# tomasjakab/imm

Hardware: AMD Instinct MI355X
Metric: training images/sec at 128x128 K=10 (higher is better)
Workload: dtype bf16; 1 GPU; BASELINE configs[1] (N>1: configs[2]): CelebA-shape 128x128 K=10 IMM training step (fwd + VGG16 perceptual loss + bwd + clip + Adam), batch 32 per GPU; global_batch=32, image_size=128, n_maps=10, parallelism=dp1, hip_graph=True, weights=seeded random init; synthetic VGG16 (vgg16.caffemodel.h5 unavailable offline)

## Files before the change

imm_amd/_lib.py:

```python
import ctypes as C
import os

import torch

_HERE = os.path.dirname(os.path.abspath(__file__))
LIB_PATH = os.environ.get('IMM_HIP_LIB') or os.path.join(_HERE, 'libimm_hip.so')

IMM_BF16, IMM_F16, IMM_F32 = 0, 1, 2
CONV_BIAS, CONV_RELU, CONV_STATS, CONV_MASK, CONV_OUT_F32 = 1, 2, 4, 8, 16
SSE_BLOCKS = 512
OPTIMIZERS = {'adam': 0, 'adadelta': 1, 'adagrad': 2}
GAUSS_MODES = {'rot': 0, 'flat': 1, 'ankush': 2}
ABI_VERSION = 25


class ImmHipError(RuntimeError):
    pass


class ConvDesc(C.Structure):
    _fields_ = [(n, C.c_int32) for n in (
        'batch', 'hi', 'wi', 'ci', 'ldx', 'ho', 'wo', 'co', 'ldy', 'kh', 'kw', 'stride', 'pad_t', 'pad_l',
        'updiv', 'kpad', 'flags', 'ldmask', 'out_scale', 'out_off_y', 'out_off_x')]


class WgradJob(C.Structure):
    _fields_ = [('desc', ConvDesc), ('x', C.c_void_p), ('dy', C.c_void_p), ('slab', C.c_void_p), ('lddy', C.c_int32),
                ('nsplit', C.c_int32), ('x_scale', C.c_void_p), ('x_shift', C.c_void_p), ('x_relu', C.c_int32),
# ... 97 lines not shown
    'imm_masked_sse': [_P, _P, _I, _I, _I, _I, _P, _I, _I, _P, _P],
    'imm_masked_sse_f32': [_P, _I, _P, _I, _I, _I, _I, _P, _I, _P, _P],
    'imm_perceptual_finalize': [_P, _I, _P, _P, _I, _P, _I, _I, _P, _P, _P],
    'imm_cost_ema': [_P, _P, _F, _P],
    'imm_rms16': [_P, _L, _I, _P, _I, _P, _P],
    'imm_tap_grad': [_P, _I, _P, _P, _I, _I, _I, _I, _P, _I, _P, _I, _I, _I, _P],
    'imm_weight_decay_loss': [_P, _P, _P, _P, _I, _P, _P, _P, _P],
    'imm_clip_adam_step': [_P, _P, _P, _P, _P, _P, _P, _I, _I, _P, _P, _P, _P, _P, _P, _P, C.POINTER(OptHParams), _P, _P],
}

_SIGS_ALIGN = {
    'imm_align_coeffs': [_P, _P, _I, _I, _I, _P, _P],
    'imm_align_warp_u8': [_P, _I, _P, _P, _I, _P, _P, _P, _P, _I, _I, _I, _I, _P, _I, _P],
}

_SIGS64 = {
    'imm_conv2d_workspace_bytes': [C.POINTER(ConvDesc)],
    'imm_conv2d_group_workspace_bytes': [_P, _I],
    'imm_conv2d_wgrad_workspace_bytes': [C.POINTER(ConvDesc), _I, _I],
    'imm_conv2d_wgrad_multi_table_bytes': [_I],
    'imm_colsum_workspace_bytes': [_L, _I],
    'imm_bn_bwd_workspace_bytes': [_L, _I],
    'imm_upsample2x_bwd_bn_workspace_bytes': [_I, _I, _I, _I],
    'imm_masked_sse_workspace_bytes': [_I],
    'imm_vgg_head_scratch_bytes': [_I, _I],
}

_lib = None


def declared_symbols():
    return sorted(list(_SIGS) + list(_SIGS64) + ['imm_last_error', 'imm_source_digest'])


def alignment_symbols():
    return sorted(_SIGS_ALIGN)


def load():
    global _lib
    if _lib is not None:
        return _lib
    if not os.path.exists(LIB_PATH):
        raise ImmHipError('libimm_hip.so not found at %s: build it with `python imm_amd/build.py` '
                          '(there is no CPU fallback for the product path)' % LIB_PATH)
    if 'IMM_HIP_LIB' not in os.environ and os.path.isdir(os.path.join(_HERE, 'csrc')):
        from . import build as _b
        want, have = _b.source_digest(), _b.library_digest(LIB_PATH)
        if want != have:
            if not _b.have_compiler():
                raise ImmHipError('libimm_hip.so is stale (built from sources %s.., checkout is %s..) and hipcc is not '
                                  'available to rebuild it' % (have[:12] or '?', want[:12]))
            _b.build(verbose=False)
    lib = C.CDLL(LIB_PATH)
    for name in ('imm_last_error', 'imm_source_digest'):
        getattr(lib, name).restype = C.c_char_p
        getattr(lib, name).argtypes = []
    for name, args in list(_SIGS.items()) + list(_SIGS_ALIGN.items()):
        fn = getattr(lib, name)
        fn.argtypes = args
        fn.restype = C.c_int
    for name, args in _SIGS64.items():
        fn = getattr(lib, name)
        fn.argtypes = args
        fn.restype = C.c_int64
    v = lib.imm_abi_version()
    if v != ABI_VERSION:
        raise ImmHipError('libimm_hip.so ABI %d != expected %d' % (v, ABI_VERSION))
    _lib = lib
    return lib


def check(rc, what):
# ... 9 lines not shown
```

imm_amd/csrc/conv_common.h:

```cpp
#pragma once
#include "common.h"

struct ConvArgs {
  const uint16_t* x;
  const uint16_t* wt;
  const float* bias;
  void* y;
  float* stats;
  const uint16_t* mask;
  int M, hi, wi, ci8, ldx;
  int ho, wo, co, ldy;
  int kh, kw, stride, pad_t, pad_l, updiv;
  int kpad, KT, ntaps;
  int flags, ldmask;
  int n_nblk, n_blocks;
  int oscale, ooff_y, ooff_x;
  uint32_t x_bytes, wt_bytes;
  const uint16_t* tap_gt;
  const float* tap_lmask;
  const float* tap_coef;
  int tap_idx, tap_S, tap_l1;
};
#define IMM_CONV_TAP_ 0x20


#define IMM_CONV_GROUP_MAX 4
struct ConvArgsGroup {
  ConvArgs a[IMM_CONV_GROUP_MAX];
  int first[IMM_CONV_GROUP_MAX + 1];
  int n;
};

template <typename ET, int BM, int BN, int WGM, int WGN, int MT, int NT>
__device__ __forceinline__ void conv_epilogue(const ConvArgs& a, f32x4_t (&acc)[MT][NT], int tid, int wm, int wn, int m0,
                                              int n0, int mblk, float* red) {
  constexpr int TM = BM / WGM, TN = BN / WGN;
  const int lane = tid & 63;
  if (a.flags & IMM_DBG_NO_EPILOGUE) {
// ... 119 lines not shown
```

imm_amd/csrc/conv_hdeep.hip:

```cpp
#include "conv_common.h"
#include <stdlib.h>
#include <stdio.h>

typedef __attribute__((address_space(3))) void lds_void_t;
typedef __attribute__((ext_vector_type(4))) unsigned int u32x4_t;

#define HD_PW 16
#define HD_HW (HD_PW + 2)
#define HD_SLOTS(PH) (((PH) + 2) * HD_HW)
#define HD_HINSTR(PH) ((HD_SLOTS(PH) + 7) / 8)
#define HD_HSTAGE(PH) (HD_HINSTR(PH) * 64)
#define HD_OOB 0x80000000u

struct HdArgs {
  ConvArgs c;
  int n_patches, patches_x, patches_y;
  int n_wg;
  int n_img;
  unsigned long long* prof;
};

__device__ __forceinline__ void hd_dma16(u32x4_t rsrc, uint32_t lds_addr, uint32_t voff, uint32_t soff) {
  asm volatile("s_mov_b32 m0, %0\n\ts_nop 0\n\tbuffer_load_dwordx4 %1, %2, %3 offen lds"
               :: "s"(lds_addr), "v"(voff), "s"(rsrc), "s"(soff) : "memory");
// ... 7 lines not shown
template <int V> struct HdInt { static constexpr int value = V; };

__device__ __forceinline__ float hd_row_sum16(float x) {
  float y;
  asm volatile("s_nop 1\n\tv_add_f32_dpp %0, %1, %1 row_ror:8 row_mask:0xf bank_mask:0xf\n\t"
               "s_nop 1\n\tv_add_f32_dpp %0, %0, %0 row_ror:4 row_mask:0xf bank_mask:0xf\n\t"
               "s_nop 1\n\tv_add_f32_dpp %0, %0, %0 row_ror:2 row_mask:0xf bank_mask:0xf\n\t"
               "s_nop 1\n\tv_add_f32_dpp %0, %0, %0 row_ror:1 row_mask:0xf bank_mask:0xf\n\ts_nop 1"
               : "=&v"(y) : "v"(x));
  return y;
}

#ifndef IMM_HD_ROLL
#define IMM_HD_ROLL 1
#endif
template <typename ET, int BN, int NW, int PH, bool MAP8 = false, int NSB_ = 0, bool PERSIST = false, bool ROW3 = false, bool S2D = false>
__global__ __launch_bounds__(NW * 64) void conv_hdeep_kernel(const HdArgs ha) {
  const ConvArgs& a = ha.c;
  constexpr bool COL = IMM_HD_ROLL && ROW3 && !S2D && !MAP8;
  static_assert(!S2D || (!MAP8 && !PERSIST && NW == 4 && BN == 64), "stride-2 data gradient: 8x16 class patches x 64 channels, one tile per workgroup");
  constexpr int NCLS = S2D ? 4 : 1;
  static_assert((NW == 8 && PH == 16) || (NW == 4 && PH == 8), "wave (wm, wn) owns patch rows 4wm..4wm+3 x BN/2 channels");
  static_assert(!MAP8 || NW == 4, "two 8x8 images per 4-wave workgroup");
  static_assert(!(PERSIST && MAP8), "persistent tiles: 16x16 / 8x16 patches only");
  static_assert(!ROW3 || (NSB_ == 9 && !PERSIST), "row-at-a-time schedule: nine tap stages, one tile per workgroup");
  constexpr int HD_NSB = NSB_ ? NSB_ : MAP8 ? 3 : 4;
  constexpr int NPIECE = MAP8 ? 7 : 6;
  constexpr int TN = BN / 2, MT = 4, NT = TN / 16;
  constexpr int B_I = BN / (8 * NW);
  constexpr int SLOTS = MAP8 ? 200 : HD_SLOTS(PH);
  constexpr int HINSTR = (SLOTS + 7) / 8, HSTAGE = HINSTR * 64;
  static_assert(B_I >= 1 && NPIECE * NW >= HINSTR && (ROW3 || NPIECE <= 11 - HD_NSB), "halo pieces per wave cover the halo and land in time");
  constexpr int STEP_I = MAP8 ? 160 : (HD_HW * 128) / 16, STEP_KY = MAP8 ? 80 : (HD_HW * 128) / 16;
// ... 261 lines not shown
      ++t;
    }
  }
  HD_STAMP(4);
  if (!have_next) {
    asm volatile("s_waitcnt lgkmcnt(0)" ::: "memory");
    asm volatile("s_waitcnt vmcnt(0)" ::: "memory");
    __syncthreads();
  } else {
    asm volatile("s_waitcnt vmcnt(0)" ::: "memory");
  }
  HD_STAMP(5);
  const int img = e_img, y0 = e_y0, x0 = e_x0, n0 = e_n0, patch = e_patch;

  const bool f_relu = a.flags & IMM_CONV_RELU;
  const bool f_stats = !PERSIST && (a.flags & IMM_CONV_STATS), f_mask = a.flags & IMM_CONV_MASK;
  const int nb = n0 + wn * TN + q * (4 * NT);
  float s1[NT][4], s2[NT][4];
#pragma unroll
  for (int j = 0; j < NT; ++j)
#pragma unroll
    for (int r = 0; r < 4; ++r) { s1[j][r] = 0.f; s2[j][r] = 0.f; }
  if (have_next) load_bias(n_n0);
  const int64_t m_first = MAP8 ? ((int64_t)(img + wm) * 8 + (frow >> 3)) * 8 + (frow & 7)
                               : ((int64_t)img * a.ho + y0 + wm * 4) * a.wo + x0 + frow;
  const int64_t m_step = MAP8 ? 16 : a.wo;
  const bool rows_exist = !MAP8 || img + wm < ha.n_img;
  typedef short s16x2_t __attribute__((ext_vector_type(2)));
  typedef unsigned short u16x2_t __attribute__((ext_vector_type(2)));
  const s16x2_t zero2 = {0, 0}, one2 = {1, 1};
  if constexpr (S2D) {
// ... 36 lines not shown
          const int j = 2 * h + (e >> 1), r = (e & 1) * 2;
          v[2 * e] = acc[0][i][j][r]; v[2 * e + 1] = acc[0][i][j][r + 1];
        }
        unpack8<ET>(*(const uint4*)(a.mask + m * a.ldmask + nb + 8 * h), fp);
        unpack8<ET>(*(const uint4*)(a.tap_gt + m * a.ldmask + nb + 8 * h), fg);
#pragma unroll
        for (int e = 0; e < 8; ++e) {
          float d = fp[e] - fg[e];
          if (a.tap_l1) d = d > 0.f ? 1.f : (d < 0.f ? -1.f : 0.f);
          float t = ET::to_f32(ET::from_f32(v[e])) + cm * d;
          if (!(fp[e] > 0.f)) t = 0.f;
          v[e] = t;
        }
        *(uint4*)((uint16_t*)a.y + m * a.ldy + nb + 8 * h) = pack8<ET>(v);
      }
    }
  } else if (!f_stats && rows_exist) {
#pragma unroll
    for (int i = 0; i < MT; ++i) {
      const int64_t m = m_first + i * m_step;
#pragma unroll
      for (int h = 0; h < NT / 2; ++h) {
        uint32_t w[4];
#pragma unroll
        for (int e = 0; e < 4; ++e) {
          const int j = 2 * h + (e >> 1), r = (e & 1) * 2;
          w[e] = ET::pack2(acc[0][i][j][r], acc[0][i][j][r + 1]);
        }
        if (f_relu) {
#pragma unroll
// ... 138 lines not shown
  if (off) return false;
  if (d->kh != 3 || d->kw != 3 || d->stride != 1 || d->updiv != 1 || d->pad_t != 1 || d->pad_l != 1) return false;
  if (d->ci % 64 || d->co % 64 || d->ci < 64) return false;
  if (d->out_scale > 1 || (d->flags & (IMM_CONV_OUT_F32 | 0xf00))) return false;
  if (d->hi != d->ho || d->wi != d->wo || d->ho % 8 || (d->wo % HD_PW && !(d->ho == 8 && d->wo == 8))) return false;
  if (d->ldy % 8 || ((d->flags & IMM_CONV_MASK) && d->ldmask % 8)) return false;
  const int64_t px = (int64_t)d->batch * d->hi * d->wi;
  if (px * d->ldx * 2 >= (1LL << 31) || (int64_t)d->co * d->kpad * 2 >= (1LL << 31)) return false;
  constexpr int min_wg = 100;
  const HdPlan p = hd_plan(d);
  return p.n_patches > 0 && p.n_wg >= min_wg;
}

int imm_hdeep_stats_blocks(const imm_conv_desc* d) { return hd_plan(d).n_patches; }

static bool hd_takes_hdeep6(const imm_conv_desc* d, const HdPlan& p);
int imm_hdeep_variant(const imm_conv_desc* d) {
  const HdPlan p = hd_plan(d);
  if (hd_takes_hdeep6(d, p)) return 600000 + (p.persist ? 1 : 0);
  const bool one_wave = p.n_wg <= hd_num_cu();
  const bool row3 = (p.map8 && one_wave) || (p.ph == 8 && p.bn == 64 && !p.map8 && one_wave) || (p.ph == 16 && p.bn == 64 && p.row3);
  const bool persist = !row3 && !p.map8 && p.ph == 16 && p.persist;
  return 500000 + (p.map8 ? 40000 : 0) + (row3 ? 20000 : 0) + (persist ? 10000 : 0) + p.bn * 10 + (p.ph == 16 ? 8 : 4);
}

template <typename ET, int BN, int NW, int PH, bool MAP8 = false, int NSB_ = 0, bool PERSIST = false, bool ROW3 = false, bool S2D = false>
static void hd_launch_cfg(const HdArgs& ha, hipStream_t s) {
  constexpr int hstage = MAP8 ? 25 * 64 : HD_HSTAGE(PH), nsb = NSB_ ? NSB_ : MAP8 ? 3 : 4;
  constexpr int lds = (2 * hstage + 64 + nsb * BN * 8) * 16 + (PERSIST ? NW * BN * 4 : 0);
  static bool attr_set = false;
  if (!attr_set) {
    (void)hipFuncSetAttribute((const void*)conv_hdeep_kernel<ET, BN, NW, PH, MAP8, NSB_, PERSIST, ROW3, S2D>, hipFuncAttributeMaxDynamicSharedMemorySize, lds);
    attr_set = true;
  }
  const int grid = PERSIST ? (ha.n_wg < hd_num_cu() ? ha.n_wg : hd_num_cu()) : ha.n_wg;
  hipLaunchKernelGGL((conv_hdeep_kernel<ET, BN, NW, PH, MAP8, NSB_, PERSIST, ROW3, S2D>), dim3(grid), dim3(NW * 64), lds, s, ha);
}

template <typename ET>
static void hd_launch(const HdPlan& p, const HdArgs& ha, hipStream_t s) {
  constexpr bool row3 = true;
  const bool one_wave = p.n_wg <= hd_num_cu();
  if (p.map8 && row3 && one_wave) hd_launch_cfg<ET, 64, 4, 8, true, 9, false, true>(ha, s);
  else if (p.ph == 8 && p.bn == 64 && !p.map8 && row3 && one_wave) hd_launch_cfg<ET, 64, 4, 8, false, 9, false, true>(ha, s);
  else if (p.map8) hd_launch_cfg<ET, 64, 4, 8, true>(ha, s);
  else if (p.ph == 16 && p.bn == 128 && p.persist) hd_launch_cfg<ET, 128, 8, 16, false, 0, true>(ha, s);
  else if (p.ph == 16 && p.bn == 128) hd_launch_cfg<ET, 128, 8, 16>(ha, s);
  else if (p.ph == 16 && p.bn == 64 && p.row3) hd_launch_cfg<ET, 64, 8, 16, false, 9, false, true>(ha, s);
  else if (p.ph == 16 && p.persist) hd_launch_cfg<ET, 64, 8, 16, false, 0, true>(ha, s);
  else if (p.ph == 16) hd_launch_cfg<ET, 64, 8, 16>(ha, s);
  else hd_launch_cfg<ET, 64, 4, 8>(ha, s);
}

static unsigned long long* hd_prof_buf = nullptr;
static void hd_prof_dump() {
  if (!hd_prof_buf) return;
  static unsigned long long host[4000];
  if (hipDeviceSynchronize() != hipSuccess || hipMemcpy(host, hd_prof_buf, sizeof(host), hipMemcpyDeviceToHost) != hipSuccess) return;
  const int n = (int)host[0] < 4000 ? (int)host[0] : 4000;
  const unsigned long long mask = 0xffffffffffffffull;
  for (int i = 1; i < n; ++i)
    fprintf(stderr, "HDPROF %4d code %d  t %9.2f us  (+%7.2f)\n", i, (int)(host[i] >> 56), (double)((host[i] & mask) - (host[1] & mask)) / 100.0,
            i > 1 ? (double)((host[i] & mask) - (host[i - 1] & mask)) / 100.0 : 0.0);
}

bool imm_hdeep6_enabled();
// ... 10 lines not shown
  if (prof && !hd_prof_buf && hipMalloc((void**)&hd_prof_buf, 4000 * sizeof(unsigned long long)) == hipSuccess) {
    (void)hipMemset(hd_prof_buf, 0, 4000 * sizeof(unsigned long long));
    atexit(hd_prof_dump);
  }
  ha.prof = prof ? hd_prof_buf : nullptr;
  const HdPlan p = hd_plan(d);
  ha.patches_x = p.map8 ? 1 : d->wo / HD_PW; ha.patches_y = p.map8 ? 1 : d->ho / p.ph;
  ha.n_img = d->batch;
  ha.n_patches = p.n_patches;
  ha.c.n_nblk = d->co / p.bn;
  ha.n_wg = p.n_wg;
  ha.c.x_bytes = (uint32_t)((int64_t)d->batch * d->hi * d->wi * d->ldx * 2);
  ha.c.wt_bytes = (uint32_t)((int64_t)d->co * d->kpad * 2);
  if (hd_takes_hdeep6(d, p)) {
    imm_conv_hdeep6_launch(dtype, ha.c, ha.n_patches, ha.patches_x, ha.patches_y, ha.n_wg, p.persist, hd_num_cu(), s);
    return;
  }
  if (dtype == IMM_BF16) hd_launch<BF16>(p, ha, s); else hd_launch<F16>(p, ha, s);
}

bool imm_hdeep_s2d_applicable(const imm_conv_desc* d) {
  static const bool off = imm_conv_disabled("s2d");
  if (off) return false;
  if (d->kh != 3 || d->kw != 3 || d->stride != 1 || d->updiv != 1 || d->pad_t != 1 || d->pad_l != 1) return false;
  if (d->ci % 64 || d->ci < 64 || d->ldx != d->ci || d->kpad != 9 * d->ci) return false;
  if (d->co % 8 || d->co < 8 || d->ldy % 8 || d->ldy < d->co) return false;
  if (d->hi != d->ho || d->wi != d->wo || d->ho % 8 || d->wo % HD_PW) return false;
  if (d->flags || d->out_scale > 1) return false;
  const int64_t px = (int64_t)d->batch * d->hi * d->wi;
  if (px * d->ldx * 2 >= (1LL << 31) || (int64_t)d->co * d->kpad * 2 >= (1LL << 31)) return false;
// ... 25 lines not shown
```

imm_amd/csrc/conv_igemm.hip:

```cpp
#include "conv_common.h"
#include <stdlib.h>

bool imm_halo_applicable(const imm_conv_desc* d);
int imm_halo_grid(const imm_conv_desc* d);
void imm_conv_halo_launch(int dtype, const imm_conv_desc* d, const ConvArgs& a, hipStream_t s);
bool imm_hdeep_applicable(const imm_conv_desc* d);
int imm_hdeep_stats_blocks(const imm_conv_desc* d);
int imm_hdeep_variant(const imm_conv_desc* d);
void imm_conv_hdeep_launch(int dtype, const imm_conv_desc* d, const ConvArgs& a, hipStream_t s);
bool imm_halo_nol_applicable(const imm_conv_desc* d);
void imm_conv_halo_nol_launch(int dtype, const imm_conv_desc* d, const ConvArgs& a, const float* scale, const float* shift, int relu,
                              hipStream_t s);
bool imm_halo_s2d_applicable(const imm_conv_desc* d);
void imm_conv_halo_s2d_launch(int dtype, const imm_conv_desc* d, const ConvArgs& a, hipStream_t s);
bool imm_s2f_applicable(const imm_conv_desc* d);
int imm_s2f_stats_blocks(const imm_conv_desc* d);
int imm_s2f_variant(const imm_conv_desc* d);
void imm_conv_s2f_launch(int dtype, const imm_conv_desc* d, const ConvArgs& a, hipStream_t s);
bool imm_hdeep_s2d_applicable(const imm_conv_desc* d);
void imm_conv_hdeep_s2d_launch(int dtype, const imm_conv_desc* d, const ConvArgs& a, hipStream_t s);
bool imm_halo2_applicable(const imm_conv_desc* d);
int imm_halo2_grid(const imm_conv_desc* d);
bool imm_halo2_x32(const imm_conv_desc* d);
void imm_conv_halo2_launch(int dtype, const imm_conv_desc* d, const ConvArgs& a, hipStream_t s);
// ... 251 lines not shown
void imm_conv64_launch(int dtype, ConvArgs& a, int bm, int bn, hipStream_t s);
bool imm_conv64_group_launch(int dtype, ConvArgs* args, int n, int bm, int bn, hipStream_t s);

static void fill_args(ConvArgs& a, const imm_conv_desc* d, const void* x, const void* wt, const float* bias, void* y,
                      float* stats, const void* mask) {
  a.x = (const uint16_t*)x; a.wt = (const uint16_t*)wt; a.bias = bias; a.y = y; a.stats = stats;
  a.mask = (const uint16_t*)mask;
  a.M = d->batch * d->ho * d->wo;
  a.hi = d->hi; a.wi = d->wi; a.ci8 = d->ci / 8; a.ldx = d->ldx;
  a.ho = d->ho; a.wo = d->wo; a.co = d->co; a.ldy = d->ldy;
  a.kh = d->kh; a.kw = d->kw; a.stride = d->stride; a.pad_t = d->pad_t; a.pad_l = d->pad_l; a.updiv = d->updiv;
  a.kpad = d->kpad; a.KT = d->kpad / 32; a.ntaps = d->kh * d->kw;
  a.flags = d->flags; a.ldmask = d->ldmask;
  a.oscale = d->out_scale > 1 ? d->out_scale : 1; a.ooff_y = d->out_off_y; a.ooff_x = d->out_off_x;
  a.tap_gt = nullptr; a.tap_lmask = nullptr; a.tap_coef = nullptr; a.tap_idx = 0; a.tap_S = 0; a.tap_l1 = 0;
}

template <typename ET>
static int conv_launch(const imm_conv_desc* d, const void* x, const void* wt, const float* bias, void* y,
                       float* stats, const void* mask, hipStream_t s) {
  ConvArgs a;
  fill_args(a, d, x, wt, bias, y, stats, mask);
  if (imm_halo2_applicable(d)) {
    imm_conv_halo2_launch(ET::kEnum, d, a, s);
    IMM_CHECK_LAUNCH("imm_conv2d(halo2)");
    return 0;
  }
  if (imm_halo_applicable(d)) {
    imm_conv_halo_launch(ET::kEnum, d, a, s);
    IMM_CHECK_LAUNCH("imm_conv2d(halo)");
// ... 70 lines not shown
  IMM_REQUIRE(d && x && wt && y && a_pred && a_gt && coef && idx >= 0, "conv_tap: null");
  if (!imm_conv2d_tap_supported(d)) return imm_fail(IMM_E_UNSUPPORTED, "conv_tap: shape not served by the LDS-halo deep-K kernel");
  IMM_REQUIRE(lda >= d->co && lda % 8 == 0, "conv_tap: lda=%d (co=%d) must be a multiple of 8", lda, d->co);
  IMM_REQUIRE(loss_mask == nullptr || (S >= d->ho && S % d->ho == 0 && d->ho == d->wo), "conv_tap: mask side");
  IMM_REQUIRE(((uintptr_t)x % 16 == 0) && ((uintptr_t)wt % 16 == 0) && ((uintptr_t)y % 16 == 0) && ((uintptr_t)a_pred % 16 == 0) &&
                  ((uintptr_t)a_gt % 16 == 0), "conv_tap: 16-byte alignment");
  IMM_REQUIRE(dtype == IMM_BF16 || dtype == IMM_F16, "unknown dtype %d", dtype);
  imm_conv_desc dd = *d;
  dd.ldmask = lda;
  ConvArgs a;
  fill_args(a, &dd, x, wt, nullptr, y, nullptr, a_pred);
  a.flags |= IMM_CONV_TAP_;
  a.tap_gt = (const uint16_t*)a_gt; a.tap_lmask = loss_mask; a.tap_coef = coef; a.tap_idx = idx; a.tap_S = S; a.tap_l1 = l1;
  imm_conv_hdeep_launch(dtype, &dd, a, (hipStream_t)stream);
  IMM_CHECK_LAUNCH("imm_conv2d_tap");
  return 0;
}

extern "C" int imm_conv2d_nol_supported(const imm_conv_desc* d) {
  if (!d || validate_desc(d)) return 0;
  if (d->flags & (IMM_CONV_MASK | IMM_CONV_RELU | 0xfe0)) return 0;
  return imm_halo_nol_applicable(d) ? 1 : 0;
}

extern "C" int imm_conv2d_nol_stats_blocks(const imm_conv_desc* d) {
  if (!imm_conv2d_nol_supported(d)) return imm_fail(IMM_E_UNSUPPORTED, "conv_nol: shape not served by the LDS-halo kernel");
  return imm_halo_grid(d);
}

extern "C" int imm_conv2d_nol(const imm_conv_desc* d, int dtype, const void* x_raw, const float* x_scale, const float* x_shift,
// ... 186 lines not shown
```

imm_amd/engine.py:

```python
import math
import os
from collections import OrderedDict

import numpy as np
import torch

from . import _lib as L
from . import ops

BN_EPS = 1e-3
BN_MOMENTUM = 0.99
BN_DIRECT_ROWS = int(os.environ.get('IMM_BN_DIRECT_ROWS', '512'))
WEIGHT_DECAY = 1e-5
INIT_STD = 0.01
PERCEPTUAL_WS = [100.0, 1.6, 2.3, 1.8, 2.8, 100.0]
SUPPORTED_COMP = ['input', 'conv1_2', 'conv2_2', 'conv3_2', 'conv4_2', 'conv5_2']
VGG_LAYERS = [('conv1_1', 1, 64), ('conv1_2', 64, 64), ('conv2_1', 64, 128), ('conv2_2', 128, 128),
              ('conv3_1', 128, 256), ('conv3_2', 256, 256), ('conv3_3', 256, 256),
              ('conv4_1', 256, 512), ('conv4_2', 512, 512), ('conv4_3', 512, 512),
              ('conv5_1', 512, 512), ('conv5_2', 512, 512)]
VGG_POOL_AFTER = ('conv1_2', 'conv2_2', 'conv3_3', 'conv4_3')
WGRAD_MULTI_MAX_JOBS, WGRAD_MULTI_MAX_VARIANTS = 64, 16


# ... 855 lines not shown
        for name, cin, cout in self.vgg_layers[1:]:
            fd = self.vgg_desc[name]
            wm = w['vgg16/%s/weights' % name]
            ops.pack_weights(wm, self.vgg_wt[name], 0, 3, 3, cin, cout, cin, self.vgg_wt[name].shape[0], fd.kpad)
            wtd = self.vgg_wtd[name]
            ops.pack_weights(wm, wtd, 1, 3, 3, cin, cout, cout, wtd.shape[0], wtd.shape[1])

    def _build_backward(self):
        B, S, K, dt, Cj = self.B, self.S, self.K, self.dt, self.Cj
        mask = self.in_mask
        acts = self.vgg_act
        l1 = self.l1
        names = [n for n, _ci, _co in self.vgg_layers]
        taps = self.tap_idx
        dbuf = {n: self._act(B, acts[n][1], acts[n][1], acts[n][0].shape[-1]) for n in names}
        dpool = {n: self._act(B, acts[n][1] // 2, acts[n][1] // 2, acts[n][0].shape[-1]) for n in self.vgg_pool}

        def pred_half(t):
            return t[B:]

        def tap(name, has_in):
            y, H = acts[name]
            c = y.shape[-1]
            self._add(self.prog_bwd, lambda: ops.tap_grad(dbuf[name], has_in, y[B:], y[:B], B, H, c, mask, S, self.coef,
                                                          taps[name], True, l1), 'tap_grad', 0.0, B * H * H * c * 8.0)

        fused_taps = set()

        def dgrad(name, dst, mask_ref, tap_of=None):
            cin, cout = [(ci, co) for n, ci, co in VGG_LAYERS if n == name][0]
            H = acts[name][1]
# ... 18 lines not shown
        def unpool(src_name, dy, relu_mask):
            y, H = acts[src_name]
            c = y.shape[-1]
            self._add(self.prog_bwd, lambda: ops.maxpool2_bwd(y[B:], dy, dbuf[src_name], B, H, H, c, relu_mask), 'maxpool_bwd',
                      0.0, B * H * H * c * 5.0)

        def unpool_tap(name, dy):
            if l1:
                unpool(name, dy, 0); tap(name, True)
                return
            y, H = acts[name]
            c = y.shape[-1]
            self._add(self.prog_bwd, lambda: ops.unpool_tap_grad(dbuf[name], dy, y[B:], y[:B], B, H, c, mask, S, self.coef,
                                                                 taps[name]), 'tap_grad', 0.0, B * H * H * c * 8.5)

        for i in range(len(names) - 1, 0, -1):
            name, prev = names[i], names[i - 1]
            deepest = i == len(names) - 1
            if name in self.vgg_pool:
                if name in taps:
                    unpool_tap(name, dpool[name])
                else:
                    unpool(name, dpool[name], 1)
            elif name in taps and name not in fused_taps:
                tap(name, not deepest)
            if prev in self.vgg_pool:
                dgrad(name, dpool[prev], None)
            elif prev in taps:
                dgrad(name, dbuf[prev], None, tap_of=prev)
            else:
                dgrad(name, dbuf[prev], pred_half(acts[prev][0]))
        last = self.ren[-1]
        self.d_pred = self._act(B, S, S, last.lddy)
        in_idx = taps.get('input', -1)
        if names:
            self._add(self.prog_bwd, lambda: ops.vgg_conv1_1_bwd(dbuf['conv1_1'], B, S, self.w11, self.in_future, self.pred,
                                                                 self.ldp, mask, self.coef, self.d_pred, last.lddy, in_idx, l1),
                      'vgg_conv1_1_bwd', 2.0 * B * S * S * 9 * 64)
        else:
            self._add(self.prog_bwd, lambda: ops.image_loss_grad(self.in_future, self.pred, self.ldp, B, S, mask, self.coef, in_idx,
                                                                 self.d_pred, last.lddy, l1), 'image_loss_grad')

        ups = {idx: (ub, H, co) for idx, ub, H, co in self.ren_up}
        d_out, ldd = self.d_pred, last.lddy
        up_src = None
        for i in range(len(self.ren) - 1, -1, -1):
            lay = self.ren[i]
            if i == 0:
                dx, lddx = self.d_joint, Cj
            else:
                prev = self.ren[i - 1]
                if (i - 1) in ups:
                    _ub, Hp, cp = ups[i - 1]
# ... 288 lines not shown
```

imm_amd/ops.py:

```python
import ctypes as C

import torch

from . import _lib as L
from ._lib import ConvDesc, OptHParams, call


def _s():
    return C.c_void_p(torch.cuda.current_stream().cuda_stream)


def _p(t):
    if t is None:
        return None
    return C.c_void_p(t.data_ptr())


def dtype_enum(dt):
    if dt == torch.bfloat16:
        return L.IMM_BF16
    if dt == torch.float16:
        return L.IMM_F16
    if dt == torch.float32:
        return L.IMM_F32
# ... 120 lines not shown
def wgrad_reduce_multi(tab):
    call('imm_wgrad_reduce_multi', _p(tab.jobs), _p(tab.blk_first), tab.n_jobs, tab.n_blocks, _s())


def conv2d(desc, x, wt, bias, y, stats=None, mask=None):
    call('imm_conv2d', C.byref(desc), dtype_enum(x.dtype), _p(x), _p(wt), _p(bias), _p(y), _p(stats), _p(mask), _s())


def conv2d_tap_supported(desc):
    return bool(L.load().imm_conv2d_tap_supported(C.byref(desc)))


def conv2d_tap(desc, x, wt, y, a_pred, a_gt, lda, loss_mask, S, coef, idx, l1=False):
    call('imm_conv2d_tap', C.byref(desc), dtype_enum(x.dtype), _p(x), _p(wt), _p(y), _p(a_pred), _p(a_gt), lda, _p(loss_mask), S,
         _p(coef), idx, int(l1), _s())


def conv_stats_blocks(desc):
    n = L.load().imm_conv_stats_blocks(C.byref(desc))
    if n <= 0:
        raise L.ImmHipError('imm_conv_stats_blocks: ' + L.load().imm_last_error().decode())
    return n


def conv2d_wgrad(desc, x, dy, lddy, slab, nsplit):
    call('imm_conv2d_wgrad', C.byref(desc), dtype_enum(x.dtype), _p(x), _p(dy), lddy, _p(slab), nsplit, _s())


CONV_FAMILIES = {1: 'igemm', 2: 'igemm64', 3: 'halo', 4: 'halo2', 5: 'hdeep', 6: 'hdeep6', 7: 's2f', 8: 'f32'}

# ... 569 lines not shown
```

include/imm_hip.h:

```cpp
#ifndef IMM_HIP_H
#define IMM_HIP_H

#include <stdint.h>

#ifdef __cplusplus
extern "C" {
#endif

#define IMM_ABI_VERSION 25

enum imm_dtype { IMM_BF16 = 0, IMM_F16 = 1, IMM_F32 = 2 };

enum imm_error {
  IMM_OK = 0,
  IMM_E_INVALID = -1,
  IMM_E_UNSUPPORTED = -2,
  IMM_E_HIP = -3
};

#define IMM_CONV_BIAS 1
#define IMM_CONV_RELU 2
#define IMM_CONV_STATS 4
#define IMM_CONV_MASK 8
#define IMM_CONV_OUT_F32 16
// ... 219 lines not shown
int imm_tps_warp_pad(const float* src, int ld_src, int batch, int h, int w, int c, int pad_y, int pad_x, int grid_h, int grid_w,
                     int crop_y, int crop_x, int out_h, int out_w, const float* basis_t, int m3, const float* w_tps,
                     float* dst, int ld_dst, void* stream);

int imm_resize_crop_u8(const uint8_t* src, const int64_t* offsets, const int32_t* hw, const int32_t* boxes, int batch, int c,
                       int resize_h, int resize_w, int crop_y0, int crop_x0, int out_h, int out_w, float* dst, int ld_dst,
                       void* stream);


int imm_crc32c(const void* data, uint64_t n, uint32_t* crc_inout);

#ifdef __cplusplus
}
#endif
#include "imm_align.h"
#endif
```

Before: 10300 images/s.

## Fuse max-pool backward (unpool) and tap gradient into VGG dgrad conv epilogue

Adds an UNPOOL epilogue to the deep-K LDS-halo conv kernel. The data-gradient conv feeding a pooled VGG layer now scatters its output straight to the 2x2 argmax position, recomputing the argmax from the forward activations. It also optionally applies the ReLU mask or adds the perceptual-tap gradient. This removes the intermediate pooled-gradient buffer and the separate unpool/tap_grad kernels, so there is less launch overhead and memory traffic. In exchange the epilogue does more work and more scattered stores, and it only covers 64-channel stride-1 shapes.

```diff
diff --git a/imm_amd/_lib.py b/imm_amd/_lib.py
--- a/imm_amd/_lib.py
+++ b/imm_amd/_lib.py
@@ -11,7 +11,7 @@
 SSE_BLOCKS = 512
 OPTIMIZERS = {'adam': 0, 'adadelta': 1, 'adagrad': 2}
 GAUSS_MODES = {'rot': 0, 'flat': 1, 'ankush': 2}
-ABI_VERSION = 25
+ABI_VERSION = 26
 
 
 class ImmHipError(RuntimeError):
@@ -139,6 +139,11 @@
     'imm_align_warp_u8': [_P, _I, _P, _P, _I, _P, _P, _P, _P, _I, _I, _I, _I, _P, _I, _P],
 }
 
+_SIGS_VGG_BWD = {
+    'imm_conv2d_unpool_supported': [C.POINTER(ConvDesc)],
+    'imm_conv2d_unpool': [C.POINTER(ConvDesc), _I, _P, _P, _P, _P, _P, _I, _I, _P, _I, _P, _I, _P],
+}
+
 _SIGS64 = {
     'imm_conv2d_workspace_bytes': [C.POINTER(ConvDesc)],
     'imm_conv2d_group_workspace_bytes': [_P, _I],
@@ -160,6 +165,10 @@
 
 def alignment_symbols():
     return sorted(_SIGS_ALIGN)
+
+
+def vgg_bwd_symbols():
+    return sorted(_SIGS_VGG_BWD)
 
 
 def load():
@@ -181,7 +190,7 @@
     for name in ('imm_last_error', 'imm_source_digest'):
         getattr(lib, name).restype = C.c_char_p
         getattr(lib, name).argtypes = []
-    for name, args in list(_SIGS.items()) + list(_SIGS_ALIGN.items()):
+    for name, args in list(_SIGS.items()) + list(_SIGS_ALIGN.items()) + list(_SIGS_VGG_BWD.items()):
         fn = getattr(lib, name)
         fn.argtypes = args
         fn.restype = C.c_int
diff --git a/imm_amd/csrc/conv_common.h b/imm_amd/csrc/conv_common.h
--- a/imm_amd/csrc/conv_common.h
+++ b/imm_amd/csrc/conv_common.h
@@ -20,8 +20,10 @@
   const float* tap_lmask;
   const float* tap_coef;
   int tap_idx, tap_S, tap_l1;
+  int unpool_relu;
 };
 #define IMM_CONV_TAP_ 0x20
+#define IMM_CONV_UNPOOL_ 0x40
 
 
 #define IMM_CONV_GROUP_MAX 4
diff --git a/imm_amd/csrc/conv_hdeep.hip b/imm_amd/csrc/conv_hdeep.hip
--- a/imm_amd/csrc/conv_hdeep.hip
+++ b/imm_amd/csrc/conv_hdeep.hip
@@ -45,9 +45,11 @@
 #ifndef IMM_HD_ROLL
 #define IMM_HD_ROLL 1
 #endif
-template <typename ET, int BN, int NW, int PH, bool MAP8 = false, int NSB_ = 0, bool PERSIST = false, bool ROW3 = false, bool S2D = false>
+template <typename ET, int BN, int NW, int PH, bool MAP8 = false, int NSB_ = 0, bool PERSIST = false, bool ROW3 = false, bool S2D = false,
+          bool UNPOOL = false>
 __global__ __launch_bounds__(NW * 64) void conv_hdeep_kernel(const HdArgs ha) {
   const ConvArgs& a = ha.c;
+  static_assert(!UNPOOL || (BN == 64 && !S2D), "pooling-adjoint epilogue: 64-channel blocks of the stride-1 forms");
   constexpr bool COL = IMM_HD_ROLL && ROW3 && !S2D && !MAP8;
   static_assert(!S2D || (!MAP8 && !PERSIST && NW == 4 && BN == 64), "stride-2 data gradient: 8x16 class patches x 64 channels, one tile per workgroup");
   constexpr int NCLS = S2D ? 4 : 1;
@@ -339,7 +341,7 @@
   const int img = e_img, y0 = e_y0, x0 = e_x0, n0 = e_n0, patch = e_patch;
 
   const bool f_relu = a.flags & IMM_CONV_RELU;
-  const bool f_stats = !PERSIST && (a.flags & IMM_CONV_STATS), f_mask = a.flags & IMM_CONV_MASK;
+  const bool f_stats = !PERSIST && !UNPOOL && (a.flags & IMM_CONV_STATS), f_mask = a.flags & IMM_CONV_MASK;
   const int nb = n0 + wn * TN + q * (4 * NT);
   float s1[NT][4], s2[NT][4];
 #pragma unroll
@@ -406,6 +408,70 @@
         }
         *(uint4*)((uint16_t*)a.y + m * a.ldy + nb + 8 * h) = pack8<ET>(v);
       }
+    }
+  } else if constexpr (UNPOOL) {
+    if (rows_exist) {
+    const bool f_tap = a.tap_gt != nullptr;
+    const float ck = f_tap ? a.tap_coef[a.tap_idx] : 0.f;
+    const int H2 = 2 * a.ho, W2 = 2 * a.wo, rr = a.tap_lmask ? a.tap_S / H2 : 1;
+    const int bi = MAP8 ? img + wm : img;
+#pragma unroll
+    for (int i = 0; i < MT; ++i) {
+      const int Y = MAP8 ? 2 * i + (frow >> 3) : y0 + wm * 4 + i, X = MAP8 ? (frow & 7) : x0 + frow;
+      const int64_t p00 = ((int64_t)bi * H2 + 2 * Y) * W2 + 2 * X;
+      const int64_t pq[4] = {p00, p00 + 1, p00 + W2, p00 + W2 + 1};
+      float cm[4] = {ck, ck, ck, ck};
+      if (f_tap && a.tap_lmask) {
+#pragma unroll
+        for (int w = 0; w < 4; ++w)
+          cm[w] = ck * a.tap_lmask[((int64_t)bi * a.tap_S + (int64_t)(2 * Y + (w >> 1)) * rr) * a.tap_S + (int64_t)(2 * X + (w & 1)) * rr];
+      }
+#pragma unroll
+      for (int h = 0; h < NT / 2; ++h) {
+        float g[8], fp[4][8], o[8];
+        int am[8];
+        {
+          uint32_t gw[4];
+#pragma unroll
+          for (int e = 0; e < 4; ++e) {
+            const int j = 2 * h + (e >> 1), r = (e & 1) * 2;
+            gw[e] = ET::pack2(acc[0][i][j][r], acc[0][i][j][r + 1]);
+          }
+          unpack8<ET>(make_uint4(gw[0], gw[1], gw[2], gw[3]), g);
+        }
+#pragma unroll
+        for (int w = 0; w < 4; ++w) unpack8<ET>(*(const uint4*)(a.mask + pq[w] * a.ldmask + nb + 8 * h), fp[w]);
+#pragma unroll
+        for (int e = 0; e < 8; ++e) {
+          float mv = fp[0][e];
+          am[e] = 0;
+#pragma unroll
+          for (int w = 1; w < 4; ++w) if (fp[w][e] > mv) { mv = fp[w][e]; am[e] = w; }
+          if (!f_tap && a.unpool_relu && !(mv > 0.f)) g[e] = 0.f;
+        }
+        if (f_tap) {
+#pragma unroll
+          for (int w = 0; w < 4; ++w) {
+            float fg[8];
+            unpack8<ET>(*(const uint4*)(a.tap_gt + pq[w] * a.ldmask + nb + 8 * h), fg);
+#pragma unroll
+            for (int e = 0; e < 8; ++e) {
+              float v = ((w == am[e]) ? g[e] : 0.f) + cm[w] * (fp[w][e] - fg[e]);
+              if (!(fp[w][e] > 0.f)) v = 0.f;
+              o[e] = v;
+            }
+            *(uint4*)((uint16_t*)a.y + pq[w] * a.ldy + nb + 8 * h) = pack8<ET>(o);
+          }
+        } else {
+#pragma unroll
+          for (int w = 0; w < 4; ++w) {
+#pragma unroll
+            for (int e = 0; e < 8; ++e) o[e] = (w == am[e]) ? g[e] : 0.f;
+            *(uint4*)((uint16_t*)a.y + pq[w] * a.ldy + nb + 8 * h) = pack8<ET>(o);
+          }
+        }
+      }
+    }
     }
   } else if (!f_stats && rows_exist) {
 #pragma unroll
@@ -574,6 +640,12 @@
 
 int imm_hdeep_stats_blocks(const imm_conv_desc* d) { return hd_plan(d).n_patches; }
 
+bool imm_hdeep_unpool_applicable(const imm_conv_desc* d) {
+  static const bool off = imm_conv_disabled("unpool_epi");
+  if (off || !imm_hdeep_applicable(d)) return false;
+  return hd_plan(d).bn == 64;
+}
+
 static bool hd_takes_hdeep6(const imm_conv_desc* d, const HdPlan& p);
 int imm_hdeep_variant(const imm_conv_desc* d) {
   const HdPlan p = hd_plan(d);
@@ -584,32 +656,37 @@
   return 500000 + (p.map8 ? 40000 : 0) + (row3 ? 20000 : 0) + (persist ? 10000 : 0) + p.bn * 10 + (p.ph == 16 ? 8 : 4);
 }
 
-template <typename ET, int BN, int NW, int PH, bool MAP8 = false, int NSB_ = 0, bool PERSIST = false, bool ROW3 = false, bool S2D = false>
+template <typename ET, int BN, int NW, int PH, bool MAP8 = false, int NSB_ = 0, bool PERSIST = false, bool ROW3 = false, bool S2D = false,
+          bool UNPOOL = false>
 static void hd_launch_cfg(const HdArgs& ha, hipStream_t s) {
   constexpr int hstage = MAP8 ? 25 * 64 : HD_HSTAGE(PH), nsb = NSB_ ? NSB_ : MAP8 ? 3 : 4;
   constexpr int lds = (2 * hstage + 64 + nsb * BN * 8) * 16 + (PERSIST ? NW * BN * 4 : 0);
   static bool attr_set = false;
   if (!attr_set) {
-    (void)hipFuncSetAttribute((const void*)conv_hdeep_kernel<ET, BN, NW, PH, MAP8, NSB_, PERSIST, ROW3, S2D>, hipFuncAttributeMaxDynamicSharedMemorySize, lds);
+    (void)hipFuncSetAttribute((const void*)conv_hdeep_kernel<ET, BN, NW, PH, MAP8, NSB_, PERSIST, ROW3, S2D, UNPOOL>, hipFuncAttributeMaxDynamicSharedMemorySize, lds);
     attr_set = true;
   }
   const int grid = PERSIST ? (ha.n_wg < hd_num_cu() ? ha.n_wg : hd_num_cu()) : ha.n_wg;
-  hipLaunchKernelGGL((conv_hdeep_kernel<ET, BN, NW, PH, MAP8, NSB_, PERSIST, ROW3, S2D>), dim3(grid), dim3(NW * 64), lds, s, ha);
-}
-
-template <typename ET>
+  hipLaunchKernelGGL((conv_hdeep_kernel<ET, BN, NW, PH, MAP8, NSB_, PERSIST, ROW3, S2D, UNPOOL>), dim3(grid), dim3(NW * 64), lds, s, ha);
+}
+
+template <typename ET, bool UP = false>
 static void hd_launch(const HdPlan& p, const HdArgs& ha, hipStream_t s) {
   constexpr bool row3 = true;
   const bool one_wave = p.n_wg <= hd_num_cu();
-  if (p.map8 && row3 && one_wave) hd_launch_cfg<ET, 64, 4, 8, true, 9, false, true>(ha, s);
-  else if (p.ph == 8 && p.bn == 64 && !p.map8 && row3 && one_wave) hd_launch_cfg<ET, 64, 4, 8, false, 9, false, true>(ha, s);
-  else if (p.map8) hd_launch_cfg<ET, 64, 4, 8, true>(ha, s);
-  else if (p.ph == 16 && p.bn == 128 && p.persist) hd_launch_cfg<ET, 128, 8, 16, false, 0, true>(ha, s);
-  else if (p.ph == 16 && p.bn == 128) hd_launch_cfg<ET, 128, 8, 16>(ha, s);
-  else if (p.ph == 16 && p.bn == 64 && p.row3) hd_launch_cfg<ET, 64, 8, 16, false, 9, false, true>(ha, s);
-  else if (p.ph == 16 && p.persist) hd_launch_cfg<ET, 64, 8, 16, false, 0, true>(ha, s);
-  else if (p.ph == 16) hd_launch_cfg<ET, 64, 8, 16>(ha, s);
-  else hd_launch_cfg<ET, 64, 4, 8>(ha, s);
+  if (p.map8 && row3 && one_wave) hd_launch_cfg<ET, 64, 4, 8, true, 9, false, true, false, UP>(ha, s);
+  else if (p.ph == 8 && p.bn == 64 && !p.map8 && row3 && one_wave) hd_launch_cfg<ET, 64, 4, 8, false, 9, false, true, false, UP>(ha, s);
+  else if (p.map8) hd_launch_cfg<ET, 64, 4, 8, true, 0, false, false, false, UP>(ha, s);
+  else if (p.ph == 16 && p.bn == 128) {
+    if constexpr (!UP) {
+      if (p.persist) hd_launch_cfg<ET, 128, 8, 16, false, 0, true>(ha, s);
+      else hd_launch_cfg<ET, 128, 8, 16>(ha, s);
+    }
+  }
+  else if (p.ph == 16 && p.bn == 64 && p.row3) hd_launch_cfg<ET, 64, 8, 16, false, 9, false, true, false, UP>(ha, s);
+  else if (p.ph == 16 && p.persist) hd_launch_cfg<ET, 64, 8, 16, false, 0, true, false, false, UP>(ha, s);
+  else if (p.ph == 16) hd_launch_cfg<ET, 64, 8, 16, false, 0, false, false, false, UP>(ha, s);
+  else hd_launch_cfg<ET, 64, 4, 8, false, 0, false, false, false, UP>(ha, s);
 }
 
 static unsigned long long* hd_prof_buf = nullptr;
@@ -650,6 +727,10 @@
   ha.c.wt_bytes = (uint32_t)((int64_t)d->co * d->kpad * 2);
   if (hd_takes_hdeep6(d, p)) {
     imm_conv_hdeep6_launch(dtype, ha.c, ha.n_patches, ha.patches_x, ha.patches_y, ha.n_wg, p.persist, hd_num_cu(), s);
+    return;
+  }
+  if (a.flags & IMM_CONV_UNPOOL_) {
+    if (dtype == IMM_BF16) hd_launch<BF16, true>(p, ha, s); else hd_launch<F16, true>(p, ha, s);
     return;
   }
   if (dtype == IMM_BF16) hd_launch<BF16>(p, ha, s); else hd_launch<F16>(p, ha, s);
diff --git a/imm_amd/csrc/conv_igemm.hip b/imm_amd/csrc/conv_igemm.hip
--- a/imm_amd/csrc/conv_igemm.hip
+++ b/imm_amd/csrc/conv_igemm.hip
@@ -7,6 +7,7 @@
 bool imm_hdeep_applicable(const imm_conv_desc* d);
 int imm_hdeep_stats_blocks(const imm_conv_desc* d);
 int imm_hdeep_variant(const imm_conv_desc* d);
+bool imm_hdeep_unpool_applicable(const imm_conv_desc* d);
 void imm_conv_hdeep_launch(int dtype, const imm_conv_desc* d, const ConvArgs& a, hipStream_t s);
 bool imm_halo_nol_applicable(const imm_conv_desc* d);
 void imm_conv_halo_nol_launch(int dtype, const imm_conv_desc* d, const ConvArgs& a, const float* scale, const float* shift, int relu,
@@ -289,6 +290,7 @@
   a.flags = d->flags; a.ldmask = d->ldmask;
   a.oscale = d->out_scale > 1 ? d->out_scale : 1; a.ooff_y = d->out_off_y; a.ooff_x = d->out_off_x;
   a.tap_gt = nullptr; a.tap_lmask = nullptr; a.tap_coef = nullptr; a.tap_idx = 0; a.tap_S = 0; a.tap_l1 = 0;
+  a.unpool_relu = 0;
 }
 
 template <typename ET>
@@ -389,6 +391,38 @@
   a.tap_gt = (const uint16_t*)a_gt; a.tap_lmask = loss_mask; a.tap_coef = coef; a.tap_idx = idx; a.tap_S = S; a.tap_l1 = l1;
   imm_conv_hdeep_launch(dtype, &dd, a, (hipStream_t)stream);
   IMM_CHECK_LAUNCH("imm_conv2d_tap");
+  return 0;
+}
+
+extern "C" int imm_conv2d_unpool_supported(const imm_conv_desc* d) {
+  if (!d || validate_desc(d)) return 0;
+  if (d->flags & (IMM_CONV_BIAS | IMM_CONV_RELU | IMM_CONV_STATS | IMM_CONV_MASK | IMM_CONV_OUT_F32 | 0xfe0)) return 0;
+  if (imm_halo2_applicable(d) || imm_halo_applicable(d)) return 0;
+  if ((int64_t)d->batch * d->ho * d->wo * 4 >= (1LL << 31)) return 0;
+  return imm_hdeep_unpool_applicable(d) && d->ho == d->wo && d->ldy % 8 == 0 ? 1 : 0;
+}
+
+extern "C" int imm_conv2d_unpool(const imm_conv_desc* d, int dtype, const void* x, const void* wt, void* da, const void* a_pred,
+                                 const void* a_gt, int lda, int relu_mask, const float* loss_mask, int S, const float* coef, int idx,
+                                 void* stream) {
+  IMM_REQUIRE(d && x && wt && da && a_pred, "conv_unpool: null");
+  if (!imm_conv2d_unpool_supported(d)) return imm_fail(IMM_E_UNSUPPORTED, "conv_unpool: shape not served by the 64-channel LDS-halo deep-K tiles");
+  IMM_REQUIRE(lda >= d->co && lda % 8 == 0, "conv_unpool: lda=%d (co=%d) must be a multiple of 8", lda, d->co);
+  IMM_REQUIRE(a_gt == nullptr || (coef && idx >= 0 && !relu_mask), "conv_unpool: the tap needs its coefficient and applies its own ReLU mask");
+  IMM_REQUIRE(a_gt != nullptr || loss_mask == nullptr, "conv_unpool: loss mask without tap");
+  IMM_REQUIRE(loss_mask == nullptr || (S >= 2 * d->ho && S % (2 * d->ho) == 0), "conv_unpool: mask side");
+  IMM_REQUIRE(((uintptr_t)x % 16 == 0) && ((uintptr_t)wt % 16 == 0) && ((uintptr_t)da % 16 == 0) && ((uintptr_t)a_pred % 16 == 0) &&
+                  ((uintptr_t)a_gt % 16 == 0), "conv_unpool: 16-byte alignment");
+  IMM_REQUIRE(dtype == IMM_BF16 || dtype == IMM_F16, "unknown dtype %d", dtype);
+  imm_conv_desc dd = *d;
+  dd.ldmask = lda;
+  ConvArgs a;
+  fill_args(a, &dd, x, wt, nullptr, da, nullptr, a_pred);
+  a.flags |= IMM_CONV_UNPOOL_;
+  a.unpool_relu = relu_mask ? 1 : 0;
+  a.tap_gt = (const uint16_t*)a_gt; a.tap_lmask = a_gt ? loss_mask : nullptr; a.tap_coef = coef; a.tap_idx = idx; a.tap_S = S;
+  imm_conv_hdeep_launch(dtype, &dd, a, (hipStream_t)stream);
+  IMM_CHECK_LAUNCH("imm_conv2d_unpool");
   return 0;
 }
 
diff --git a/imm_amd/engine.py b/imm_amd/engine.py
--- a/imm_amd/engine.py
+++ b/imm_amd/engine.py
@@ -893,7 +893,12 @@
         names = [n for n, _ci, _co in self.vgg_layers]
         taps = self.tap_idx
         dbuf = {n: self._act(B, acts[n][1], acts[n][1], acts[n][0].shape[-1]) for n in names}
-        dpool = {n: self._act(B, acts[n][1] // 2, acts[n][1] // 2, acts[n][0].shape[-1]) for n in self.vgg_pool}
+        dpool = {}
+
+        def pooled_grad(n):
+            if n not in dpool:
+                dpool[n] = self._act(B, acts[n][1] // 2, acts[n][1] // 2, acts[n][0].shape[-1])
+            return dpool[n]
 
         def pred_half(t):
             return t[B:]
@@ -942,18 +947,44 @@
             self._add(self.prog_bwd, lambda: ops.unpool_tap_grad(dbuf[name], dy, y[B:], y[:B], B, H, c, mask, S, self.coef,
                                                                  taps[name]), 'tap_grad', 0.0, B * H * H * c * 8.5)
 
+        fused_pools = set()
+
+        def dgrad_unpool(name, prev):
+            cin, cout = [(ci, co) for n, ci, co in VGG_LAYERS if n == name][0]
+            H = acts[name][1]
+            ya = acts[prev][0]
+            tapped = prev in taps
+            du = ops.dgrad_desc(B, H, H, cin, cin, cout, cout, 3, 1, 0)
+            if self.f32 or (tapped and l1) or ya.shape[-1] != cin or not ops.conv2d_unpool_supported(du):
+                return False
+            wtd, src, dst = self.vgg_wtd[name], dbuf[name], dbuf[prev]
+            if tapped:
+                fn = lambda: ops.conv2d_unpool(du, src, wtd, dst, ya[B:], ya[:B], cin, 0, mask, S, self.coef, taps[prev])
+            else:
+                fn = lambda: ops.conv2d_unpool(du, src, wtd, dst, ya[B:], None, cin, 1)
+            nbytes = 2.0 * (B * H * H * (cout + 4 * cin * (3 if tapped else 2)) + 9 * cin * cout)
+            if tapped and mask is not None:
+                nbytes += 4.0 * B * 4 * H * H
+            self._add(self.prog_bwd, fn, 'vgg_dgrad', 2.0 * B * H * H * 9 * cin * cout, nbytes,
+                      name='vgg16/%s+%s(%s)' % (name, 'unpool_tap' if tapped else 'unpool', prev), desc=du)
+            fused_pools.add(prev)
+            return True
+
         for i in range(len(names) - 1, 0, -1):
             name, prev = names[i], names[i - 1]
             deepest = i == len(names) - 1
-            if name in self.vgg_pool:
+            if name in fused_pools:
+                pass
+            elif name in self.vgg_pool:
                 if name in taps:
-                    unpool_tap(name, dpool[name])
+                    unpool_tap(name, pooled_grad(name))
                 else:
-                    unpool(name, dpool[name], 1)
+                    unpool(name, pooled_grad(name), 1)
             elif name in taps and name not in fused_taps:
                 tap(name, not deepest)
             if prev in self.vgg_pool:
-                dgrad(name, dpool[prev], None)
+                if not dgrad_unpool(name, prev):
+                    dgrad(name, pooled_grad(prev), None)
             elif prev in taps:
                 dgrad(name, dbuf[prev], None, tap_of=prev)
             else:
@@ -964,7 +995,8 @@
         if names:
             self._add(self.prog_bwd, lambda: ops.vgg_conv1_1_bwd(dbuf['conv1_1'], B, S, self.w11, self.in_future, self.pred,
                                                                  self.ldp, mask, self.coef, self.d_pred, last.lddy, in_idx, l1),
-                      'vgg_conv1_1_bwd', 2.0 * B * S * S * 9 * 64)
+                      'vgg_conv1_1_bwd', 2.0 * B * S * S * 9 * 64,
+                      B * S * S * (2.0 * 64 + 2 * 3 * self.pred.element_size() + 4 + 2.0 * last.lddy))
         else:
             self._add(self.prog_bwd, lambda: ops.image_loss_grad(self.in_future, self.pred, self.ldp, B, S, mask, self.coef, in_idx,
                                                                  self.d_pred, last.lddy, l1), 'image_loss_grad')
diff --git a/imm_amd/ops.py b/imm_amd/ops.py
--- a/imm_amd/ops.py
+++ b/imm_amd/ops.py
@@ -158,6 +158,15 @@
 def conv2d_tap(desc, x, wt, y, a_pred, a_gt, lda, loss_mask, S, coef, idx, l1=False):
     call('imm_conv2d_tap', C.byref(desc), dtype_enum(x.dtype), _p(x), _p(wt), _p(y), _p(a_pred), _p(a_gt), lda, _p(loss_mask), S,
          _p(coef), idx, int(l1), _s())
+
+
+def conv2d_unpool_supported(desc):
+    return bool(L.load().imm_conv2d_unpool_supported(C.byref(desc)))
+
+
+def conv2d_unpool(desc, x, wt, da, a_pred, a_gt, lda, relu_mask, loss_mask=None, S=0, coef=None, idx=0):
+    call('imm_conv2d_unpool', C.byref(desc), dtype_enum(x.dtype), _p(x), _p(wt), _p(da), _p(a_pred), _p(a_gt), lda, int(relu_mask),
+         _p(loss_mask), S, _p(coef), idx, _s())
 
 
 def conv_stats_blocks(desc):
diff --git a/include/imm_hip.h b/include/imm_hip.h
--- a/include/imm_hip.h
+++ b/include/imm_hip.h
@@ -7,7 +7,7 @@
 extern "C" {
 #endif
 
-#define IMM_ABI_VERSION 25
+#define IMM_ABI_VERSION 26
 
 enum imm_dtype { IMM_BF16 = 0, IMM_F16 = 1, IMM_F32 = 2 };
 
@@ -257,4 +257,5 @@
 }
 #endif
 #include "imm_align.h"
+#include "imm_vgg_bwd.h"
 #endif
diff --git a/include/imm_vgg_bwd.h b/include/imm_vgg_bwd.h
--- /dev/null
+++ b/include/imm_vgg_bwd.h
@@ -0,0 +1,17 @@
+#ifndef IMM_VGG_BWD_H
+#define IMM_VGG_BWD_H
+
+#include "imm_hip.h"
+
+#ifdef __cplusplus
+extern "C" {
+#endif
+
+int imm_conv2d_unpool_supported(const imm_conv_desc* desc_host);
+int imm_conv2d_unpool(const imm_conv_desc* desc_host, int dtype, const void* x, const void* wt, void* da, const void* a_pred,
+                      const void* a_gt, int lda, int relu_mask, const float* loss_mask, int S, const float* coef, int idx, void* stream);
+
+#ifdef __cplusplus
+}
+#endif
+#endif
```

Result: no change. 10220 images/s (-0.7%).
